# krm01/Snappy.jl

Measured on AMD Instinct MI355X. Metric: GB/s compressed+decompressed (batched blocks) at 1/2/4/8 GPUs; % HBM peak, higher is better.
Workload: dtype u8; 1 GPU; configs 2+3: 10000 x 64 KiB text blocks per GPU, fast-mode compress + uncompress round trip per step; blocks_per_gpu=10000, block_bytes=65536, parallelism=dp1 (blocks sharded per rank, RCCL size all-gather)

## Files before the change

snappy.jl_amd/csrc/sm_compress_sc.hip:

```cpp
#include "sm_device.h"
#include "sm_internal.h"

namespace sm {

constexpr uint32_t kScS = 1024;
constexpr uint32_t kScC = kScS / 64;
constexpr uint32_t kScG = kScS / 64;
constexpr uint32_t kScW = 16;
constexpr uint32_t kScWorkers = kScW - 1;
#ifndef SC_RING
#define SC_RING 16
#endif
constexpr uint32_t kScRing = SC_RING;
static_assert((kScRing & (kScRing - 1)) == 0, "the span kernel's slot sequence needs a power of 2");
constexpr uint32_t kScSlot = 1088;
constexpr uint32_t kScThreads = 64 * kScW;
constexpr uint32_t kScTabBits = 13;
constexpr uint32_t kScTabWords = 1u << kScTabBits;
constexpr uint32_t kScExt = 17;
constexpr uint32_t kScMaxL = 255;
#ifndef SC_SPIN_BITS
#define SC_SPIN_BITS 22
#endif
constexpr uint32_t kScSpinMax = 1u << SC_SPIN_BITS;
static_assert(kScC == 16 && kScG == 16, "a lane's 16 positions: one u16 mask, one 16-byte row");

#ifndef SC_CB
#define SC_CB 2
#endif
#ifndef SC_FAR
#define SC_FAR 256
#endif
constexpr uint32_t kMaskPasses = 16;
#ifndef SC_WPRIO
#define SC_WPRIO 3
#endif
#ifndef SC_TPRIO
#define SC_TPRIO 3
#endif
#ifndef SC_TSLEEP
#define SC_TSLEEP 1
#endif
#ifndef SC_WSLEEP
#define SC_WSLEEP 1
#endif


struct ScWaveLds {
  uint8_t L[kScS];
  uint16_t O[kScS];
};
struct ScLds {
  uint8_t pre[16];
  uint8_t blk[kBlockSize + 64];
  uint32_t T[kScTabWords + 4];
  ScWaveLds w[kScWorkers];
  uint8_t ring[kScRing][kScSlot];
  uint32_t rsize[kScRing];
  uint32_t rseq[kScRing];
  uint32_t ins;
  uint32_t next;
  uint32_t err;
};
static_assert(sizeof(ScLds) <= 160 * 1024, "LDS");
static_assert(sizeof(ScWaveLds) % 32 == 0 && offsetof(ScLds, w) % 32 == 0 && offsetof(ScWaveLds, O) % 32 == 0,
              "rows are 32-byte aligned (section C's O addresses XOR the swizzle into bits 2..4)");
static_assert(kScSlot % 16 == 0 && offsetof(ScLds, ring) % 16 == 0, "slots are 16-byte aligned");
static_assert(kScSlot == kSpanSlot, "the host sizes part pitches by the staging slot");

template <typename Pred>
__device__ __attribute__((always_inline)) inline uint32_t sc_wait(uint32_t* p, Pred pred, uint32_t& err, uint32_t code) {
  uint32_t v;
  for (uint32_t it = 0; !pred(v = uniform(__hip_atomic_load(p, __ATOMIC_ACQUIRE, __HIP_MEMORY_SCOPE_WORKGROUP))); ++it) {
    if (it > kScSpinMax) {
      err |= code;
      break;
    }
    if (SC_WSLEEP) __builtin_amdgcn_s_sleep(SC_WSLEEP);
  }
  return v;
}


__device__ inline uint32_t sc_ld32(const uint8_t* blk, uint32_t a) { return *reinterpret_cast<const uint32_t*>(blk + a); }


__device__ inline uint32_t sc_abyte(uint32_t hi, uint32_t lo, uint32_t s) { return __builtin_amdgcn_alignbyte(hi, lo, s); }

__device__ inline uint32_t sc_ld32u(const uint8_t* blk, uint32_t p) {
  const uint32_t* w = reinterpret_cast<const uint32_t*>(blk + (p & ~3u));
  return sc_abyte(w[1], w[0], p);
}

__device__ inline uint4 sc_ld128(const uint8_t* blk, uint32_t p) {
  const uint32_t* w = reinterpret_cast<const uint32_t*>(blk + (p & ~3u));
  const uint32_t s = p;
  const uint32_t w0 = w[0], w1 = w[1], w2 = w[2], w3 = w[3], w4 = w[4];
  return make_uint4(__builtin_amdgcn_alignbyte(w1, w0, s), __builtin_amdgcn_alignbyte(w2, w1, s),
                    __builtin_amdgcn_alignbyte(w3, w2, s), __builtin_amdgcn_alignbyte(w4, w3, s));
}

__device__ inline uint32_t sc_diff8(uint32_t a0, uint32_t a1, uint32_t b0, uint32_t b1) {
  const uint64_t d = ((uint64_t)(a1 ^ b1) << 32) | (a0 ^ b0);
  return d ? (uint32_t)__builtin_ctzll(d) >> 3 : 8u;
}

__device__ inline uint4 sc_trim(uint4 v, uint32_t len) {
  const uint64_t mlo = len >= 8 ? ~0ull : (1ull << (8 * (len & 7))) - 1;
  const uint64_t mhi = len >= 16 ? ~0ull : (len <= 8 ? 0ull : (1ull << (8 * (len & 7))) - 1);
  return make_uint4(v.x & (uint32_t)mlo, v.y & (uint32_t)(mlo >> 32), v.z & (uint32_t)mhi, v.w & (uint32_t)(mhi >> 32));
}

__device__ inline uint4 sc_trim1(uint4 v, uint32_t len) {
  uint32_t l8 = len << 3;
  asm("" : "+v"(l8));
  uint64_t mlo, mhi;
  asm("v_lshrrev_b64 %0, %1, -1" : "=v"(mlo) : "v"(64 - min(l8, 64u)));
  asm("v_lshrrev_b64 %0, %1, -1" : "=v"(mhi) : "v"(128 - l8));
  const bool hi = len > 8;
  return make_uint4(v.x & (uint32_t)mlo, v.y & (uint32_t)(mlo >> 32), hi ? v.z & (uint32_t)mhi : 0u,
                    hi ? v.w & (uint32_t)(mhi >> 32) : 0u);
}

__device__ inline void sc_lds_or(uint32_t a, uint4 v) {
  const uint32_t wa = (a - 1u) & ~3u, t = 0u - a;
  const uint32_t u0 = __builtin_amdgcn_alignbyte(v.x, 0u, t);
  const uint32_t u1 = __builtin_amdgcn_alignbyte(v.y, v.x, t);
  const uint32_t u2 = __builtin_amdgcn_alignbyte(v.z, v.y, t);
  const uint32_t u3 = __builtin_amdgcn_alignbyte(v.w, v.z, t);
  const uint32_t u4 = __builtin_amdgcn_alignbyte(0u, v.w, t);
  asm volatile("ds_or_b32 %0, %1\nds_or_b32 %0, %2 offset:4\nds_or_b32 %0, %3 offset:8\nds_or_b32 %0, %4 offset:12\n"
               "ds_or_b32 %0, %5 offset:16"
               : : "v"(wa), "v"(u0), "v"(u1), "v"(u2), "v"(u3), "v"(u4) : "memory");
}

__device__ inline void sc_lds_orn(uint32_t a, uint4 v, uint32_t nb) {
  const uint32_t wa = (a - 1u) & ~3u, t = 0u - a, d = a - wa;
  const uint32_t u0 = __builtin_amdgcn_alignbyte(v.x, 0u, t);
  const uint32_t u1 = __builtin_amdgcn_alignbyte(v.y, v.x, t);
  asm volatile("ds_or_b32 %0, %1" : : "v"(wa), "v"(u0) : "memory");
  asm volatile("ds_or_b32 %0, %1 offset:4" : : "v"(wa), "v"(u1) : "memory");
  if (d + nb > 8) {
    const uint32_t u2 = __builtin_amdgcn_alignbyte(v.z, v.y, t);
    const uint32_t u3 = __builtin_amdgcn_alignbyte(v.w, v.z, t);
    const uint32_t u4 = __builtin_amdgcn_alignbyte(0u, v.w, t);
    asm volatile("ds_or_b32 %0, %1 offset:8\nds_or_b32 %0, %2 offset:12\nds_or_b32 %0, %3 offset:16"
                 : : "v"(wa), "v"(u2), "v"(u3), "v"(u4) : "memory");
  }
}

__device__ inline void sc_lds_or3(uint32_t a, uint32_t cv) {
  const uint32_t wa = (a - 1u) & ~3u, t = 0u - a;
  const uint32_t lo = __builtin_amdgcn_alignbyte(cv, 0u, t), hi = __builtin_amdgcn_alignbyte(0u, cv, t);
  asm volatile("ds_or_b32 %0, %1\nds_or_b32 %0, %2 offset:4" : : "v"(wa), "v"(lo), "v"(hi) : "memory");
}

__device__ inline uint4 sc_prepend(uint4 v, uint32_t tag, uint32_t t) {
  if (t == 0) return v;
  const uint32_t s = 4 - t;
  return make_uint4(__builtin_amdgcn_alignbyte(v.x, tag << (8 * s), s), __builtin_amdgcn_alignbyte(v.y, v.x, s),
                    __builtin_amdgcn_alignbyte(v.z, v.y, s), __builtin_amdgcn_alignbyte(v.w, v.z, s));
}

__device__ inline TagBytes sc_run_tag(uint32_t len) {
  __builtin_assume(len >= 1 && len <= kScS);
  return literal_tag(len, kLiteralStd);
}

__device__ inline uint32_t sc_hash_bucket(uint32_t w) {
  uint32_t h;
  asm("v_bfe_u32 %0, %1, %2, %3" : "=v"(h) : "v"(w * kHashMul), "n"(32 - kScTabBits), "n"(kScTabBits));
  return h;
}

__device__ inline uint32_t sc_select(uint64_t m, uint32_t a, uint32_t b) {
  uint32_t r;
  asm("v_cndmask_b32_e64 %0, %1, %2, %3" : "=v"(r) : "v"(b), "v"(a), "s"(m));
  return r;
}

__device__ inline uint32_t sc_sel(uint32_t c, uint32_t a, uint32_t b) { return c ? a : b; }

__device__ inline uint32_t sc_extend(const uint8_t* blk, uint32_t q, uint32_t off, uint32_t L, uint32_t cap) {
  for (;;) {
    const uint4 x = sc_ld128(blk, q + L), y = sc_ld128(blk, q + L - off);
    const uint32_t f0 = sc_diff8(x.x, x.y, y.x, y.y);
    const uint32_t fb = f0 < 8 ? f0 : 8u + sc_diff8(x.z, x.w, y.z, y.w);
    L = min(L + fb, cap);
    if (fb < 16 || L >= cap) return L;
  }
}

__device__ inline uint32_t sc_ffbl(uint32_t x) {
  uint32_t r;
  asm("v_ffbl_b32 %0, %1" : "=v"(r) : "v"(x));
  return r;
}

__device__ __attribute__((always_inline)) inline uint32_t sc_eq16(uint32_t X0, uint32_t X1, uint32_t X2, uint32_t X3,
                                                                  const uint32_t* w, uint32_t s) {
  const uint32_t a0 = w[0], a1 = w[1], a2 = w[2], a3 = w[3], a4 = w[4];
  const uint32_t b0 = sc_ffbl(X0 ^ __builtin_amdgcn_alignbyte(a1, a0, s));
  const uint32_t b1 = sc_ffbl(X1 ^ __builtin_amdgcn_alignbyte(a2, a1, s)) | 32u;
  const uint32_t b2 = sc_ffbl(X2 ^ __builtin_amdgcn_alignbyte(a3, a2, s)) | 64u;
  const uint32_t b3 = sc_ffbl(X3 ^ __builtin_amdgcn_alignbyte(a4, a3, s)) | 96u;
  return min(min(b0, b1), min(min(b2, b3), 128u)) >> 3;
}


__device__ __attribute__((always_inline)) inline uint32_t sc_eq12x(const uint8_t* blk, uint32_t x, uint32_t y) {
  const uint32_t* a = reinterpret_cast<const uint32_t*>(blk + (x & ~3u));
  const uint32_t* b = reinterpret_cast<const uint32_t*>(blk + (y & ~3u));
  const uint32_t a0 = a[0], a1 = a[1], a2 = a[2], a3 = a[3];
  const uint32_t b0 = b[0], b1 = b[1], b2 = b[2], b3 = b[3];
  const uint32_t f0 = sc_ffbl(sc_abyte(a1, a0, x) ^ sc_abyte(b1, b0, y));
  const uint32_t f1 = sc_ffbl(sc_abyte(a2, a1, x) ^ sc_abyte(b2, b1, y)) | 32u;
  const uint32_t f2 = sc_ffbl(sc_abyte(a3, a2, x) ^ sc_abyte(b3, b2, y)) | 64u;
  return min(min(f0, f1), min(f2, 104u)) >> 3;
}

__device__ inline uint32_t scan_max_dpp(uint32_t v) {
  v = max(v, (uint32_t)__builtin_amdgcn_update_dpp(0u, v, 0x111, 0xf, 0xf, true));
  v = max(v, (uint32_t)__builtin_amdgcn_update_dpp(0u, v, 0x112, 0xf, 0xf, true));
  v = max(v, (uint32_t)__builtin_amdgcn_update_dpp(0u, v, 0x114, 0xf, 0xf, true));
  v = max(v, (uint32_t)__builtin_amdgcn_update_dpp(0u, v, 0x118, 0xf, 0xf, true));
  v = max(v, (uint32_t)__builtin_amdgcn_update_dpp(0u, v, 0x142, 0xa, 0xf, false));
  v = max(v, (uint32_t)__builtin_amdgcn_update_dpp(0u, v, 0x143, 0xc, 0xf, false));
  return v;
}

__device__ inline uint32_t sc_bits(uint32_t a, uint32_t b) { return ((1u << b) - 1u) & ~((1u << a) - 1u); }

struct ScToks {
  uint32_t t[4];
  uint32_t n;
};

__device__ __attribute__((always_inline)) inline uint32_t sc_next_block(const CompressArgs& a, uint32_t from, uint32_t g,
                                                                   uint32_t lane) {
  for (uint32_t b0 = from; b0 < a.nblk; b0 += 64 * g) {
    const uint32_t bb = b0 + lane * g;
    const bool todo = bb < a.nblk && (!a.screened || a.out_len[bb] == kScreenTodo);
    const uint64_t m = ballot(todo);
    if (m) return b0 + ctz64(m) * g;
  }
  return a.nblk;
}

template <int kDense>
__device__ __attribute__((always_inline)) inline void sc_superchunk(ScLds& S, const uint32_t k, const uint32_t n,
                                                                   const uint32_t wave, const uint32_t lane_in) {
  uint32_t lane = lane_in;
  asm volatile("" : "+v"(lane));
  ScWaveLds& Wl = S.w[wave];
  const uint32_t sc0 = k * kScS, sce = min(sc0 + kScS, n);
  const uint32_t Tbase = lds_addr(S.T);
  uint32_t ha[kScG], hvv[kScG], wq[kScG];
  const uint32_t ql = sc0 + lane, qa = ql & ~3u, qb = ql;
  const uint32_t hv0 = ql, hv1 = ql << 16;
#pragma unroll
  for (int g = 0; g < (int)kScG; ++g) {
    const uint32_t w = sc_abyte(sc_ld32(S.blk, qa + 64 * g + 4), sc_ld32(S.blk, qa + 64 * g), qb);
    wq[g] = w;
    ha[g] = Tbase + 4 * sc_hash_bucket(w);
    hvv[g] = (g & 1) ? hv1 + ((64u * g) << 16) : hv0 + 64u * g;
  }
  if (sc0 + kScS + 3 > n) {
    asm volatile("");
#pragma unroll
    for (int g = 0; g < (int)kScG; ++g) ha[g] = ql + 64 * g + 4 <= n ? ha[g] : Tbase + 4 * kScTabWords;
  }
  const uint32_t mk0 = 0xffffu, mk1 = 0xffff0000u;
  __builtin_amdgcn_s_setprio(SC_TPRIO);
  for (uint32_t it = 0; uniform(__hip_atomic_load(&S.ins, __ATOMIC_RELAXED, __HIP_MEMORY_SCOPE_WORKGROUP)) != k; ++it) {
    if (it > kScSpinMax) {
      S.err |= 1;
      break;
    }
    if (SC_TSLEEP) __builtin_amdgcn_s_sleep(SC_TSLEEP);
  }
  __builtin_amdgcn_s_setprio(3);
  const uint32_t tok_a = lds_addr(&S.ins), tok_v = k + 1;
  uint32_t r[kScG];
  asm volatile(
      "ds_mskor_rtn_b32 %0, %16, %32, %34\n"
      "ds_mskor_rtn_b32 %1, %17, %33, %35\n"
      "ds_mskor_rtn_b32 %2, %18, %32, %36\n"
      "ds_mskor_rtn_b32 %3, %19, %33, %37\n"
      "ds_mskor_rtn_b32 %4, %20, %32, %38\n"
      "ds_mskor_rtn_b32 %5, %21, %33, %39\n"
      "ds_mskor_rtn_b32 %6, %22, %32, %40\n"
      "ds_mskor_rtn_b32 %7, %23, %33, %41\n"
      "ds_mskor_rtn_b32 %8, %24, %32, %42\n"
      "ds_mskor_rtn_b32 %9, %25, %33, %43\n"
      "ds_mskor_rtn_b32 %10, %26, %32, %44\n"
      "ds_mskor_rtn_b32 %11, %27, %33, %45\n"
      "ds_mskor_rtn_b32 %12, %28, %32, %46\n"
      "ds_mskor_rtn_b32 %13, %29, %33, %47\n"
      "ds_mskor_rtn_b32 %14, %30, %32, %48\n"
      "ds_mskor_rtn_b32 %15, %31, %33, %49\n"
      "ds_write_b32 %50, %51\n"
      "s_waitcnt lgkmcnt(0)"
      : "=&v"(r[0]), "=&v"(r[1]), "=&v"(r[2]), "=&v"(r[3]), "=&v"(r[4]), "=&v"(r[5]), "=&v"(r[6]), "=&v"(r[7]),
        "=&v"(r[8]), "=&v"(r[9]), "=&v"(r[10]), "=&v"(r[11]), "=&v"(r[12]), "=&v"(r[13]), "=&v"(r[14]), "=&v"(r[15])
      : "v"(ha[0]), "v"(ha[1]), "v"(ha[2]), "v"(ha[3]), "v"(ha[4]), "v"(ha[5]), "v"(ha[6]), "v"(ha[7]), "v"(ha[8]),
        "v"(ha[9]), "v"(ha[10]), "v"(ha[11]), "v"(ha[12]), "v"(ha[13]), "v"(ha[14]), "v"(ha[15]), "v"(mk0), "v"(mk1),
        "v"(hvv[0]), "v"(hvv[1]), "v"(hvv[2]), "v"(hvv[3]), "v"(hvv[4]), "v"(hvv[5]), "v"(hvv[6]), "v"(hvv[7]),
        "v"(hvv[8]), "v"(hvv[9]), "v"(hvv[10]), "v"(hvv[11]), "v"(hvv[12]), "v"(hvv[13]), "v"(hvv[14]), "v"(hvv[15]),
        "v"(tok_a), "v"(tok_v)
      : "memory");
  __builtin_amdgcn_s_setprio(0);

  uint64_t mbs[kScG];
  uint8_t* const Ob8 = reinterpret_cast<uint8_t*>(Wl.O);
  const uint32_t Orel = 32 * (lane >> 4) + 2 * (lane & 15);
  if constexpr (kDense) {
#pragma unroll
    for (int g = 0; g < (int)kScG; ++g) {
      const uint32_t q = sc0 + 64 * g + lane;
      const uint32_t sh = 16 * (g & 1);
      const uint32_t ca = (r[g] >> sh) & 0xffffu, cb = (r[g] >> (16 - sh)) & 0xffffu;
      const uint32_t c1 = max(ca, cb), c2 = min(ca, cb);
      const bool ok1 = c1 < q;
      const uint32_t d1 = q - c1, d2 = q - c2;
      uint16_t* const Og = reinterpret_cast<uint16_t*>(Ob8 + (Orel ^ (4u * (g & 7))) + 128u * g);
      const uint32_t r4 = 4 * g + (lane >> 4), i = lane & 15;
      const uint4 X = sc_ld128(S.blk, q);
      uint32_t lw1 = sc_eq16(X.x, X.y, X.z, X.w, reinterpret_cast<const uint32_t*>(S.blk + (c1 & ~3u)), c1);
      uint32_t lw2 = sc_eq16(X.x, X.y, X.z, X.w, reinterpret_cast<const uint32_t*>(S.blk + (c2 & ~3u)), c2);
      asm("" : "+v"(lw1), "+v"(lw2));
      const uint32_t l1 = ok1 ? lw1 : 0u, l2 = ok1 ? lw2 : 0u;
      const bool take2 = l2 == l1 ? (l2 >= 4 && d1 < (uint32_t)SC_FAR) : l2 > l1;
      const uint32_t l = take2 ? l2 : l1;
      const uint32_t avail = sce - q;
      const uint32_t enc = l < 4 ? 0u : ((l == 16 && avail > 16) ? kScExt : min(l, avail));
      *Og = (uint16_t)(take2 ? d2 : d1);
      Wl.L[16 * r4 + 4 * ((i >> 2) ^ ((g >> 1) & 3)) + (i & 3)] = (uint8_t)enc;
      mbs[g] = ballot(l >= 4);
    }
  } else {
#pragma unroll
    for (int g0 = 0; g0 < (int)kScG; g0 += SC_CB) {
      uint32_t c1s[SC_CB], c2s[SC_CB], v1s[SC_CB], v2s[SC_CB];
#pragma unroll
      for (int j = 0; j < SC_CB; ++j) {
        const int g = g0 + j;
        const uint32_t sh = 16 * (g & 1);
        const uint32_t ca = (r[g] >> sh) & 0xffffu, cb = (r[g] >> (16 - sh)) & 0xffffu;
        c1s[j] = max(ca, cb);
        c2s[j] = min(ca, cb);
        v1s[j] = sc_ld32u(S.blk, c1s[j]);
        v2s[j] = sc_ld32u(S.blk, c2s[j]);
      }
#pragma unroll
      for (int j = 0; j < SC_CB; ++j) asm("" : "+v"(v1s[j]), "+v"(v2s[j]));
#pragma unroll
      for (int j = 0; j < SC_CB; ++j) {
        const int g = g0 + j;
        const uint32_t q = sc0 + 64 * g + lane;
        const uint32_t c1 = c1s[j], c2 = c2s[j], w = wq[g];
        const bool ok1 = c1 < q;
        const uint32_t d1 = q - c1, d2 = q - c2;
        uint16_t* const Og = reinterpret_cast<uint16_t*>(Ob8 + (Orel ^ (4u * (g & 7))) + 128u * g);
        const uint64_t OK = ballot(ok1);
        const uint64_t M1 = ballot(v1s[j] == w) & OK, M2 = ballot(v2s[j] == w) & OK;
        const uint64_t U = M2 & (~M1 | ballot(d1 < (uint32_t)SC_FAR));
        *Og = (uint16_t)sc_select(U, d2, d1);
        mbs[g] = M1 | M2;
      }
    }
  }
  uint32_t mdw = 0;
#define SC_WL(g)                                                                                  \
  asm volatile("v_writelane_b32 %0, %1, %2" : "+v"(mdw) : "s"((uint32_t)mbs[g]), "n"(2 * (g)));   \
  asm volatile("v_writelane_b32 %0, %1, %2" : "+v"(mdw) : "s"((uint32_t)(mbs[g] >> 32)), "n"(2 * (g) + 1));
  SC_WL(0) SC_WL(1) SC_WL(2) SC_WL(3) SC_WL(4) SC_WL(5) SC_WL(6) SC_WL(7)
  SC_WL(8) SC_WL(9) SC_WL(10) SC_WL(11) SC_WL(12) SC_WL(13) SC_WL(14) SC_WL(15)
#undef SC_WL
  __atomic_signal_fence(__ATOMIC_SEQ_CST);

  const uint32_t c0 = sc0 + kScC * lane;
  const uint32_t ce = c0 < sce ? min(c0 + kScC, sce) : c0;
  const uint32_t nroom = c0 + 3 < sce ? min(sce - c0 - 3, 16u) : 0u;
  const uint32_t mask16 = (__shfl(mdw, (int)(lane >> 1), 64) >> (16 * (lane & 1))) & ((1u << nroom) - 1u);
  const uint32_t osw2 = ((lane >> 2) & 7) << 1, lsw4 = ((lane >> 3) & 3) << 2;
  const uint16_t* const Orow = Wl.O + 16 * lane;
  auto offAt = [&](uint32_t i) -> uint32_t { return Orow[i ^ osw2]; };
  uint8_t* const Lrow = Wl.L + 16 * lane;
  uint32_t xpos = 16, xlen = 0;
  auto walk = [&](auto kStop, uint32_t sr, uint32_t stop, uint32_t& path, uint32_t& mpos, uint32_t& pend)
      __attribute__((always_inline)) {
    const uint32_t m0 = sr < 16 ? mask16 >> sr : 0u;
    uint32_t i = sr + sc_ffbl(m0);
    path = 0;
    mpos = 16;
    uint32_t last = 16, lastL = 0;
    bool act = m0 != 0;
    while (act) {
      if constexpr (decltype(kStop)::value) {
        if ((stop >> i) & 1u) {
          mpos = i;
          break;
        }
      }
      path |= 1u << i;
      last = i;
      uint32_t enc;
      if constexpr (kDense) {
        enc = Lrow[i ^ lsw4];
      } else {
        const uint32_t q = c0 + i, off = offAt(i);
        const uint32_t p = q - off;
        enc = min(4u + sc_eq12x(S.blk + 4, q, p), sce - q);
        Lrow[i ^ lsw4] = (uint8_t)enc;
      }
      lastL = enc;
      const uint32_t t = i + min(enc, 16u);
      const uint32_t m = mask16 >> t;
      i = t + sc_ffbl(m);
      act = m != 0;
    }
    pend = ce;
    if (last < 16) {
      uint32_t L = lastL;
      const bool ext = L == kScExt;
      if (last + min(L, 16u) >= 16) {
        if (ballot(ext)) {
          if (ext) {
            if (xpos != last) {
              xlen = sc_extend(S.blk, c0 + last, offAt(last), 16u, min(kScMaxL, sce - (c0 + last)));
              xpos = last;
            }
            L = xlen;
          }
        }
        pend = c0 + last + L;
      }
    }
  };
  const bool row = c0 < sce;
  uint32_t s = c0, e, P;
  {
    uint32_t mp;
    walk(std::false_type{}, row ? 0u : 16u, 0u, P, mp, e);
    if (!row) e = c0;
  }
  for (uint32_t pass = 0;; ++pass) {
    const uint32_t pe = __builtin_amdgcn_update_dpp(0u, scan_max_dpp(e), 0x138, 0xf, 0xf, false);
    const uint32_t st = lane == 0 ? sc0 : pe;
    uint32_t sn = st;
    bool chg = st != s;
    if (!ballot(chg)) break;
    if (pass < kMaskPasses) {
      uint64_t cov = ballot(st >= ce);
      for (int it = 0; cov && it < 3; ++it) {
        const uint32_t x = sn >= ce ? 0u : e;
        const uint32_t pm = __builtin_amdgcn_update_dpp(0u, scan_max_dpp(x), 0x138, 0xf, 0xf, false);
        sn = lane == 0 ? sc0 : pm;
        const uint64_t c = ballot(sn >= ce);
        if (c == cov) break;
        cov = c;
      }
      chg = sn != s;
      if (!ballot(chg)) {
        sn = st;
        chg = st != s;
      }
    }

    const bool inrow = chg && sn < ce;
    uint32_t nP, mp, ne;
    walk(std::true_type{}, inrow ? sn - c0 : 16u, P, nP, mp, ne);
    if (chg) {
      s = sn;
      if (!inrow) {
        P = 0;
        e = sn;
      } else if (mp == 16) {
        P = nP;
        e = ne;
      } else {
        P = nP | (P & ~sc_bits(0, mp));
      }
    }
  }
  auto getL = [&](uint32_t i) -> uint32_t { return Lrow[i ^ lsw4]; };
  ScToks tk;
  {
    uint32_t pm = P;
    tk.n = (uint32_t)__builtin_popcount(P);
#pragma unroll
    for (int j = 0; j < 4; ++j) {
      const uint32_t i = pm ? (uint32_t)__builtin_ctz(pm) : 0u;
      pm &= pm - 1;
      uint32_t L = getL(i);
      L = L == kScExt ? xlen : L;
      const uint32_t off = offAt(i);
      tk.t[j] = off | (L << 16) | (i << 24);
    }
  }

  const bool live = s >= c0 && s < ce;
  uint32_t lead = 0, body = 0, trail = 0;
  {
    uint32_t p = s;
#pragma unroll
    for (int j = 0; j < 4; ++j) {
      const bool has = (uint32_t)j < tk.n;
      const uint32_t tv = tk.t[j];
      const uint32_t q = c0 + (tv >> 24), L = (tv >> 16) & 0xffu, run = q - p;
      if (j == 0)
        lead = sc_sel(has, run, 0u);
      else
        body += sc_sel(has && run, run + 1, 0u);
      body += sc_sel(has, copy_tag_bytes(tv & 0xffffu, L), 0u);
      p = sc_sel(has, q + L, p);
    }
    trail = (live && p < ce) ? ce - p : 0u;
    lead = tk.n == 0 ? trail : lead;
  }
  const uint32_t ptrail = __builtin_amdgcn_update_dpp(0u, trail, 0x138, 0xf, 0xf, false);
  const bool cont = ptrail > 0 && lead > 0;
  const bool mid = cont && tk.n == 0;
  const uint32_t Cs = scan_dpp(cont ? lead : 0u);
  const uint64_t above = ballot(!mid) & (~1ull << lane);
  const uint32_t fn = above ? ctz64(above) : 63u;
  const uint32_t Cf = __shfl(Cs, fn, 64);
  const bool starts = trail > 0 && !mid;
  const uint32_t merged = starts ? trail + Cf - Cs : 0u;
  const uint32_t mts = sc_run_tag(merged ? merged : 1u).size;
  uint32_t size;
  if (tk.n == 0)
    size = lead == 0 ? 0u : (cont ? lead : mts + trail);
  else
    size = (lead ? (cont ? lead : 1u + lead) : 0u) + body + (trail ? mts + trail : 0u);
  const uint32_t incl = scan_dpp(size);
  const uint32_t total = readlane(incl, 63);

  const uint32_t slot = k % kScRing;
  (void)sc_wait(&S.rseq[slot], [&](uint32_t v) { return v == k; }, S.err, 2u);

  uint8_t* const stg = S.ring[slot];
  {
    for (uint32_t u = lane; 16 * u < total; u += 64) reinterpret_cast<uint4*>(stg)[u] = make_uint4(0, 0, 0, 0);
    const uint32_t stga = lds_addr(stg);
    uint32_t at = incl - size, p = s;
#pragma unroll
    for (int j = 0; j < 4; ++j) {
      if ((uint32_t)j < tk.n) {
        const uint32_t tv = tk.t[j];
        const uint32_t q = c0 + (tv >> 24), L = (tv >> 16) & 0xffu, off = tv & 0xffffu;
        const uint32_t run = q - p;
        const uint32_t ts = (j == 0 && cont) ? 0u : 1u;
        const uint32_t len = run ? ts + run : 0u;
        if (ballot(len != 0)) {
          uint4 v = sc_ld128(S.blk - 4, p + 3);
          v.x = ts ? ((v.x & ~0xffu) | literal_tag1(run)) : v.x;
          if (run) sc_lds_orn(stga + at + ts - 1u, sc_trim1(v, run + 1), run + 1);
        }
        at += len;
        if (L <= 64) {
          const TagBytes c = copy_piece(off, L);
          sc_lds_or3(stga + at, (uint32_t)c.bytes);
          at += c.size;
        } else {
          uint32_t R = L;
          do {
            const uint32_t l = copy_piece_len(R);
            const TagBytes c = copy_piece(off, l);
            sc_lds_or3(stga + at, (uint32_t)c.bytes);
            at += c.size;
            R -= l;
          } while (R);
        }
        p = q + L;
      }
    }
    if (live && p < ce) {
      const uint32_t run = ce - p;
      uint32_t tag = 0, ts = 0;
      if (!(tk.n == 0 && cont)) {
        const TagBytes lt = sc_run_tag(merged);
        tag = (uint32_t)lt.bytes;
        ts = lt.size;
      }
      sc_lds_orn(stga + at, sc_trim(sc_prepend(sc_ld128(S.blk, p), tag, ts), min(ts + run, 16u)), min(ts + run, 16u));
      if (ts + run > 16) sc_lds_or(stga + at + 16, sc_trim(sc_ld128(S.blk, p + 16 - ts), ts + run - 16));
    }
  }
  __hip_atomic_store(&S.rsize[slot], total + 1, __ATOMIC_RELEASE, __HIP_MEMORY_SCOPE_WORKGROUP);
}

typedef uint32_t __attribute__((ext_vector_type(4), aligned(1))) sc_u128u;
__device__ __attribute__((always_inline)) inline void sc_copy_out(uint8_t* const g, const uint8_t* stg, uint32_t len,
                                                                 uint32_t lane) {
  const uint32_t nu = len >> 4;
  for (uint32_t u = lane; u < nu; u += 64) {
    const uint4 v = reinterpret_cast<const uint4*>(stg)[u];
    sc_u128u x;
    x.x = v.x, x.y = v.y, x.z = v.z, x.w = v.w;
    *reinterpret_cast<sc_u128u*>(g + 16 * u) = x;
  }
  if (lane < (len & 15u)) g[16 * nu + lane] = stg[16 * nu + lane];
}

__device__ __attribute__((always_inline)) inline void sc_writer(ScLds& S, uint32_t n, uint8_t* const dst, uint32_t hv,
                                                               uint32_t k0, uint32_t k1, bool whole,
                                                               uint32_t* len_out, uint32_t lane) {
  uint32_t o = hv, err = 0;
  uint32_t vpre = 0;
  for (uint32_t k = k0; k < k1; ++k) {
    const uint32_t slot = k % kScRing;
    const uint32_t sz =
        (vpre ? vpre : sc_wait(&S.rsize[slot], [](uint32_t v) { return v != 0; }, err, 4u)) - 1;
    if (err) break;
    vpre = k + 1 < k1 ? uniform(__hip_atomic_load(&S.rsize[(k + 1) % kScRing], __ATOMIC_ACQUIRE,
                                                    __HIP_MEMORY_SCOPE_WORKGROUP))
                        : 0u;
    sc_copy_out(dst + o, S.ring[slot], sz, lane);
    o += sz;
    __hip_atomic_store(&S.rsize[slot], 0u, __ATOMIC_RELAXED, __HIP_MEMORY_SCOPE_WORKGROUP);
    __hip_atomic_store(&S.rseq[slot], k + kScRing, __ATOMIC_RELEASE, __HIP_MEMORY_SCOPE_WORKGROUP);
  }
  const uint32_t len = block_literal_bytes(n, false);
  if (whole && !err && n && o > hv + len) {
    uint8_t* const g = dst + hv;
    const uint32_t tb = len - n;
    const uint32_t ad = (uint32_t)((uintptr_t)g & 15);
    uint4* const g16 = reinterpret_cast<uint4*>(g - ad);
    const uint32_t u1 = (len + ad) >> 4;
    const uint32_t ua = (tb + ad + 15) >> 4;
    for (uint32_t u = ua + lane; u < u1; u += 64) g16[u] = sc_ld128(S.blk, 16 * u - ad - tb);
    const uint32_t he = ua < u1 ? 16 * ua - ad : len;
    const uint32_t te = ua < u1 ? 16 * u1 - ad : len;
    for (uint32_t j = lane; j < he + (len - te); j += 64) {
      const uint32_t jj = j < he ? j : te + (j - he);
      g[jj] = jj < tb ? block_literal_head_byte(n, false, jj) : S.blk[jj - tb];
    }
    o = hv + len;
  }
  err |= uniform(__hip_atomic_load(&S.err, __ATOMIC_RELAXED, __HIP_MEMORY_SCOPE_WORKGROUP));
  if (lane == 0) *len_out = err ? kOutLenError | err : o;
}

__device__ __attribute__((always_inline)) inline void sc_stage_block(ScLds& S, const uint8_t* src, uint32_t n, bool there,
                                                                    uint8_t* dst, uint32_t hv) {
  const uint32_t tid = threadIdx.x;
  if (there) {
  } else if (((uintptr_t)src & 15) == 0) {
    const uint4* s16 = reinterpret_cast<const uint4*>(src);
    uint4* d16 = reinterpret_cast<uint4*>(S.blk);
    const uint32_t n16 = n >> 4;
    for (uint32_t k = tid; k < n16; k += kScThreads) d16[k] = s16[k];
    for (uint32_t k = (n & ~15u) + tid; k < n; k += kScThreads) S.blk[k] = src[k];
  } else {
    for (uint32_t k = tid; k < n; k += kScThreads) S.blk[k] = src[k];
  }
  if (tid < 64) S.blk[n + tid] = 0;
  uint4* t16 = reinterpret_cast<uint4*>(S.T);
  for (uint32_t k = tid; k < 4 * kScTabWords / 16; k += kScThreads) t16[k] = make_uint4(0, 0, 0, 0);
  if (tid < hv) dst[tid] = varint_byte(n, tid, hv);
}

__device__ __attribute__((always_inline)) inline void sc_reset_handoff(ScLds& S, uint32_t k0) {
  const uint32_t lane = threadIdx.x & 63;
  if (uniform(threadIdx.x >> 6) != 0) return;
  if (lane < kScRing) {
    S.rsize[lane] = 0;
    S.rseq[lane] = k0 + ((lane - k0) & (kScRing - 1));
  }
  if (lane == 0) {
    S.ins = k0;
    S.next = 64 * k0;
    S.err = 0;
  }
}

template <int kDense>
__device__ __attribute__((always_inline)) inline void sc_span_item(ScLds& S, const CompressArgs& a, const ScSpan& sp,
                                                                  const uint32_t item) {
  const uint32_t tid = threadIdx.x;
  const uint32_t wave = uniform(tid >> 6);
  const uint32_t lane = tid & 63;
  const uint32_t b = item / sp.parts, j = item % sp.parts;
  if (b >= a.nblk) return;
  uint32_t* const plen = sp.part_len + item;
  const uint32_t n = a.in_len[b];
  if (n > kBlockSize) {
    if (tid == 0) *plen = j == 0 ? kNotABlock : 0u;
    return;
  }
  const uint32_t nsc = (n + kScS - 1) / kScS;
  const uint32_t k0 = j * sp.span, k1 = min(k0 + sp.span, nsc);
  const bool todo = !a.screened || a.out_len[b] == kScreenTodo;
  if (!todo || k0 >= k1) {
    if (tid == 0) *plen = (!todo && j == 0) ? (sp.blk_pitch ? kPartScreened : a.out_len[b]) : 0u;
    return;
  }
  const uint8_t* const src = a.in + a.in_off[b];
  uint8_t* const dst = a.out + (sp.blk_pitch ? b * sp.blk_pitch : a.out_off[b]) + (uint64_t)j * sp.pitch;
  const uint32_t hv = (a.header && j == 0) ? varint_len(n) : 0u;
  sc_stage_block(S, src, n, false, dst, hv);
  sc_reset_handoff(S, k0);
  __syncthreads();
  const uint32_t pe = kScS * k0;
  const uint32_t sub = lane & 15, gq = lane >> 4;
  for (int ph = 1; ph >= 0; --ph) {
    for (uint32_t i = wave; 128 * (4 * i) < pe; i += kScW) {
      const uint32_t G = 2 * (4 * i + gq) + (uint32_t)ph;
      const uint32_t q = 64 * G + 4 * sub;
      if (q >= pe) continue;
      const uint32_t d0 = sc_ld32(S.blk, q), d1 = sc_ld32(S.blk, q + 4);
      uint32_t* t[4];
#pragma unroll
      for (uint32_t j = 0; j < 4; ++j) {
        const uint32_t w = j ? __builtin_amdgcn_alignbyte(d1, d0, j) : d0;
        t[j] = &S.T[(w * kHashMul) >> (32 - kScTabBits)];
      }
      if (ph) {
#pragma unroll
        for (uint32_t j = 0; j < 4; ++j)
          if (q + j + 4 <= n) __hip_atomic_fetch_max(t[j], (q + j) << 16, __ATOMIC_RELAXED, __HIP_MEMORY_SCOPE_WORKGROUP);
      } else {
        uint32_t hi[4];
#pragma unroll
        for (uint32_t j = 0; j < 4; ++j) hi[j] = __hip_atomic_load(t[j], __ATOMIC_RELAXED, __HIP_MEMORY_SCOPE_WORKGROUP);
#pragma unroll
        for (uint32_t j = 0; j < 4; ++j)
          if (q + j + 4 <= n)
            __hip_atomic_fetch_max(t[j], (hi[j] & 0xffff0000u) | (q + j), __ATOMIC_RELAXED, __HIP_MEMORY_SCOPE_WORKGROUP);
      }
    }
    __syncthreads();
  }
  if (wave == kScWorkers) {
    __builtin_amdgcn_s_setprio(SC_WPRIO);
    sc_writer(S, n, dst, hv, k0, k1, false, plen, lane);
    __builtin_amdgcn_s_setprio(0);
  } else {
    for (;;) {
      const uint32_t k = uniform(__hip_atomic_fetch_add(&S.next, 1u, __ATOMIC_RELAXED, __HIP_MEMORY_SCOPE_WORKGROUP)) >> 6;
      if (k >= k1) break;
      sc_superchunk<kDense>(S, k, n, wave, lane);
    }
  }
}

template <int kDense>
__global__ __launch_bounds__(kScThreads) void k_compress_sc_span(CompressArgs a, ScSpan sp) {
  __shared__ __attribute__((aligned(16))) ScLds S;
  sc_span_item<kDense>(S, a, sp, blockIdx.x);
}

template <int kDense>
__global__ __launch_bounds__(kScThreads) void k_compress_sc(CompressArgs a, uint32_t g, CompressArgs r, ScSpan sp) {
  __shared__ __attribute__((aligned(16))) ScLds S;
  if (blockIdx.x >= g) {
    sc_span_item<kDense>(S, r, sp, blockIdx.x - g);
    return;
  }
  const uint32_t tid = threadIdx.x;
  const uint32_t wave = uniform(tid >> 6);
  const uint32_t lane = tid & 63;
  static_assert(kBlockSize / 16 / kScThreads == 4, "four 16-byte pieces per thread of a full block");
  uint4 pf0, pf1, pf2, pf3;
  uint32_t b = sc_next_block(a, blockIdx.x, g, lane);
  uint32_t n = 0;
  const uint8_t* src = nullptr;
  bool inpf = false;
#define SC_FETCH(bb)                                                              \
  {                                                                               \
    n = (bb) < a.nblk ? a.in_len[bb] : 0u;                                        \
    src = (bb) < a.nblk ? a.in + a.in_off[bb] : nullptr;                          \
    inpf = (bb) < a.nblk && n == kBlockSize && ((uintptr_t)src & 15) == 0;        \
    if (inpf) {                                                                   \
      const uint4* s16 = reinterpret_cast<const uint4*>(src);                     \
      pf0 = s16[tid];                                                             \
      pf1 = s16[tid + kScThreads];                                                \
      pf2 = s16[tid + 2 * kScThreads];                                            \
      pf3 = s16[tid + 3 * kScThreads];                                            \
    }                                                                             \
  }
  SC_FETCH(b)
  while (b < a.nblk) {
    uint8_t* const dst = a.out + a.out_off[b];
    if (n > kBlockSize) {
      if (tid == 0) a.out_len[b] = kNotABlock;
      b = sc_next_block(a, b + g, g, lane);
      SC_FETCH(b)
      continue;
    }
    if (inpf) {
      uint4* d16 = reinterpret_cast<uint4*>(S.blk);
      d16[tid] = pf0;
      d16[tid + kScThreads] = pf1;
      d16[tid + 2 * kScThreads] = pf2;
      d16[tid + 3 * kScThreads] = pf3;
    }
    const uint32_t hv = a.header ? varint_len(n) : 0u;
    sc_stage_block(S, src, n, inpf, dst, hv);
    sc_reset_handoff(S, 0);
    const uint32_t bn = sc_next_block(a, b + g, g, lane);
    __syncthreads();

    const uint32_t nsc = (n + kScS - 1) / kScS;
    if (wave == kScWorkers) {
      __builtin_amdgcn_s_setprio(SC_WPRIO);
      sc_writer(S, n, dst, hv, 0, nsc, true, &a.out_len[b], lane);
      __builtin_amdgcn_s_setprio(0);
    } else {
      for (;;) {
        const uint32_t k = uniform(__hip_atomic_fetch_add(&S.next, 1u, __ATOMIC_RELAXED, __HIP_MEMORY_SCOPE_WORKGROUP)) >> 6;
        if (k >= nsc) break;
        sc_superchunk<kDense>(S, k, n, wave, lane);
      }
    }
    SC_FETCH(bn)
    __syncthreads();
    b = bn;
  }
#undef SC_FETCH
}

hipError_t launch_compress_sc_span(const CompressArgs& a, int mode, const ScSpan& sp, hipStream_t s) {
  if (sp.parts == 0 || sp.span == 0 || sp.parts * sp.span < (kBlockSize + kScS - 1) / kScS ||
      sp.pitch < (uint64_t)sp.span * kScSlot)
    return hipErrorInvalidValue;
  const uint32_t grid = a.nblk * sp.parts;
  if (grid == 0) return hipSuccess;
  if (mode == 2)
    hipLaunchKernelGGL(k_compress_sc_span<1>, dim3(grid), dim3(kScThreads), 0, s, a, sp);
  else
    hipLaunchKernelGGL(k_compress_sc_span<0>, dim3(grid), dim3(kScThreads), 0, s, a, sp);
  return hipGetLastError();
}


hipError_t launch_compress_sc_parts(const CompressArgs& a, const CompressArgs& r, const ScSpan& sp, int mode,
                                    hipStream_t s) {
  const uint32_t g = min(a.nblk, compress_grid());
  const uint32_t items = sp.parts ? r.nblk * sp.parts : 0u;
  if (items && (sp.span == 0 || sp.parts * sp.span < (kBlockSize + kScS - 1) / kScS ||
                sp.pitch < (uint64_t)sp.span * kScSlot || sp.blk_pitch < sp.parts * sp.pitch))
    return hipErrorInvalidValue;
  if (g + items == 0) return hipSuccess;
  if (mode == 2)
    hipLaunchKernelGGL(k_compress_sc<1>, dim3(g + items), dim3(kScThreads), 0, s, a, g, r, sp);
  else
    hipLaunchKernelGGL(k_compress_sc<0>, dim3(g + items), dim3(kScThreads), 0, s, a, g, r, sp);
  return hipGetLastError();
}

hipError_t launch_compress_sc(const CompressArgs& a, int mode, hipStream_t s) {
  return launch_compress_sc_parts(a, CompressArgs{}, ScSpan{}, mode, s);
}

}
```

Baseline: 411.5 GB/s.

## Publish next-block metadata via LDS record and prefetch partial blocks

The writer wave now looks up the next block's index, length and offsets and publishes them in a double-buffered LDS record with a release sequence number. Worker waves read that record after finishing their superchunks instead of each repeating the global metadata lookup, falling back to a direct lookup if the record is not ready. The register prefetch of the next block is extended to blocks shorter than 64 KiB (at least 16 bytes, 16-byte aligned) by clamping indices, and staging copies only the unaligned tail for those. This is meant to take global metadata latency off the block-to-block critical path, at the cost of more LDS state and added cross-wave ordering complexity.

```diff
diff --git a/snappy.jl_amd/csrc/sm_compress_sc.hip b/snappy.jl_amd/csrc/sm_compress_sc.hip
--- a/snappy.jl_amd/csrc/sm_compress_sc.hip
+++ b/snappy.jl_amd/csrc/sm_compress_sc.hip
@@ -50,6 +50,17 @@
   uint8_t L[kScS];
   uint16_t O[kScS];
 };
+struct ScNextRec {
+  uint32_t seq;
+  uint32_t b;
+  uint32_t n;
+  uint32_t pad;
+  uint64_t src;
+  uint64_t dst;
+};
+#ifndef SC_USE_RECORD
+#define SC_USE_RECORD 1
+#endif
 struct ScLds {
   uint8_t pre[16];
   uint8_t blk[kBlockSize + 64];
@@ -61,6 +72,7 @@
   uint32_t ins;
   uint32_t next;
   uint32_t err;
+  ScNextRec nx[2];
 };
 static_assert(sizeof(ScLds) <= 160 * 1024, "LDS");
 static_assert(sizeof(ScWaveLds) % 32 == 0 && offsetof(ScLds, w) % 32 == 0 && offsetof(ScWaveLds, O) % 32 == 0,
@@ -646,12 +658,13 @@
 __device__ __attribute__((always_inline)) inline void sc_stage_block(ScLds& S, const uint8_t* src, uint32_t n, bool there,
                                                                     uint8_t* dst, uint32_t hv) {
   const uint32_t tid = threadIdx.x;
-  if (there) {
-  } else if (((uintptr_t)src & 15) == 0) {
-    const uint4* s16 = reinterpret_cast<const uint4*>(src);
-    uint4* d16 = reinterpret_cast<uint4*>(S.blk);
-    const uint32_t n16 = n >> 4;
-    for (uint32_t k = tid; k < n16; k += kScThreads) d16[k] = s16[k];
+  if (there || ((uintptr_t)src & 15) == 0) {
+    if (!there) {
+      const uint4* s16 = reinterpret_cast<const uint4*>(src);
+      uint4* d16 = reinterpret_cast<uint4*>(S.blk);
+      const uint32_t n16 = n >> 4;
+      for (uint32_t k = tid; k < n16; k += kScThreads) d16[k] = s16[k];
+    }
     for (uint32_t k = (n & ~15u) + tid; k < n; k += kScThreads) S.blk[k] = src[k];
   } else {
     for (uint32_t k = tid; k < n; k += kScThreads) S.blk[k] = src[k];
@@ -752,6 +765,29 @@
   sc_span_item<kDense>(S, a, sp, blockIdx.x);
 }
 
+__device__ inline uint64_t sc_uniform64(uint64_t v) {
+  return ((uint64_t)uniform((uint32_t)(v >> 32)) << 32) | uniform((uint32_t)v);
+}
+
+struct ScBlkInfo {
+  uint32_t b, n;
+  uint64_t so, dof;
+};
+
+__device__ __attribute__((always_inline)) inline ScBlkInfo sc_lookup(const CompressArgs& a, uint32_t from, uint32_t g,
+                                                                    uint32_t lane) {
+  ScBlkInfo x;
+  x.b = sc_next_block(a, from, g, lane);
+  const bool has = x.b < a.nblk;
+  const uint32_t bi = has ? x.b : 0u;
+  const uint32_t n = a.in_len[bi];
+  const uint64_t so = a.in_off[bi], dof = a.out_off[bi];
+  x.n = uniform(has ? n : 0u);
+  x.so = sc_uniform64(has ? so : 0ull);
+  x.dof = sc_uniform64(has ? dof : 0ull);
+  return x;
+}
+
 template <int kDense>
 __global__ __launch_bounds__(kScThreads) void k_compress_sc(CompressArgs a, uint32_t g, CompressArgs r, ScSpan sp) {
   __shared__ __attribute__((aligned(16))) ScLds S;
@@ -764,60 +800,81 @@
   const uint32_t lane = tid & 63;
   static_assert(kBlockSize / 16 / kScThreads == 4, "four 16-byte pieces per thread of a full block");
   uint4 pf0, pf1, pf2, pf3;
-  uint32_t b = sc_next_block(a, blockIdx.x, g, lane);
-  uint32_t n = 0;
+  ScBlkInfo cur = sc_lookup(a, blockIdx.x, g, lane);
   const uint8_t* src = nullptr;
   bool inpf = false;
-#define SC_FETCH(bb)                                                              \
-  {                                                                               \
-    n = (bb) < a.nblk ? a.in_len[bb] : 0u;                                        \
-    src = (bb) < a.nblk ? a.in + a.in_off[bb] : nullptr;                          \
-    inpf = (bb) < a.nblk && n == kBlockSize && ((uintptr_t)src & 15) == 0;        \
-    if (inpf) {                                                                   \
-      const uint4* s16 = reinterpret_cast<const uint4*>(src);                     \
-      pf0 = s16[tid];                                                             \
-      pf1 = s16[tid + kScThreads];                                                \
-      pf2 = s16[tid + 2 * kScThreads];                                            \
-      pf3 = s16[tid + 3 * kScThreads];                                            \
-    }                                                                             \
-  }
-  SC_FETCH(b)
-  while (b < a.nblk) {
-    uint8_t* const dst = a.out + a.out_off[b];
+#define SC_FETCH(x)                                                                                \
+  {                                                                                                \
+    src = a.in + (x).so;                                                                           \
+    inpf = (x).b < a.nblk && (x).n <= kBlockSize && (x).n >= 16 && ((uintptr_t)src & 15) == 0;     \
+    if (inpf) {                                                                                    \
+      const uint4* s16 = reinterpret_cast<const uint4*>(src);                                      \
+      const uint32_t last = ((x).n >> 4) - 1;                                                      \
+      pf0 = s16[min(tid, last)];                                                                   \
+      pf1 = s16[min(tid + kScThreads, last)];                                                      \
+      pf2 = s16[min(tid + 2 * kScThreads, last)];                                                  \
+      pf3 = s16[min(tid + 3 * kScThreads, last)];                                                  \
+    }                                                                                              \
+  }
+  SC_FETCH(cur)
+  if (tid < 2) S.nx[tid].seq = 0;
+  uint32_t par = 0;
+  while (cur.b < a.nblk) {
+    const uint32_t b = cur.b, n = cur.n;
+    uint8_t* const dst = a.out + cur.dof;
     if (n > kBlockSize) {
       if (tid == 0) a.out_len[b] = kNotABlock;
-      b = sc_next_block(a, b + g, g, lane);
-      SC_FETCH(b)
+      cur = sc_lookup(a, b + g, g, lane);
+      SC_FETCH(cur)
       continue;
     }
     if (inpf) {
       uint4* d16 = reinterpret_cast<uint4*>(S.blk);
-      d16[tid] = pf0;
-      d16[tid + kScThreads] = pf1;
-      d16[tid + 2 * kScThreads] = pf2;
-      d16[tid + 3 * kScThreads] = pf3;
+      const uint32_t last = (n >> 4) - 1;
+      d16[min(tid, last)] = pf0;
+      d16[min(tid + kScThreads, last)] = pf1;
+      d16[min(tid + 2 * kScThreads, last)] = pf2;
+      d16[min(tid + 3 * kScThreads, last)] = pf3;
     }
     const uint32_t hv = a.header ? varint_len(n) : 0u;
     sc_stage_block(S, src, n, inpf, dst, hv);
     sc_reset_handoff(S, 0);
-    const uint32_t bn = sc_next_block(a, b + g, g, lane);
     __syncthreads();
 
     const uint32_t nsc = (n + kScS - 1) / kScS;
+    ScNextRec& R = S.nx[par];
+    ScBlkInfo nxt;
     if (wave == kScWorkers) {
+      nxt = sc_lookup(a, b + g, g, lane);
+      R.b = nxt.b;
+      R.n = nxt.n;
+      R.src = nxt.so;
+      R.dst = nxt.dof;
+      __hip_atomic_store(&R.seq, b + 1, __ATOMIC_RELEASE, __HIP_MEMORY_SCOPE_WORKGROUP);
       __builtin_amdgcn_s_setprio(SC_WPRIO);
       sc_writer(S, n, dst, hv, 0, nsc, true, &a.out_len[b], lane);
       __builtin_amdgcn_s_setprio(0);
+      SC_FETCH(nxt)
     } else {
       for (;;) {
         const uint32_t k = uniform(__hip_atomic_fetch_add(&S.next, 1u, __ATOMIC_RELAXED, __HIP_MEMORY_SCOPE_WORKGROUP)) >> 6;
         if (k >= nsc) break;
         sc_superchunk<kDense>(S, k, n, wave, lane);
       }
-    }
-    SC_FETCH(bn)
+      const uint32_t seq = uniform(__hip_atomic_load(&R.seq, __ATOMIC_ACQUIRE, __HIP_MEMORY_SCOPE_WORKGROUP));
+      if (SC_USE_RECORD && seq == b + 1) {
+        nxt.b = uniform(R.b);
+        nxt.n = uniform(R.n);
+        nxt.so = sc_uniform64(R.src);
+        nxt.dof = sc_uniform64(R.dst);
+      } else {
+        nxt = sc_lookup(a, b + g, g, lane);
+      }
+      SC_FETCH(nxt)
+    }
     __syncthreads();
-    b = bn;
+    cur = nxt;
+    par ^= 1;
   }
 #undef SC_FETCH
 }
```

Measured after the change: 414.4 GB/s (median of 6 runs). No clear change (+0.7%).
